# featureform/embeddinghub

Hardware: AMD Instinct MI355X
Metric: kNN queries/sec at recall@10>=0.95, 10Mx768 cosine, batch=1024 (higher is better)
Workload: dtype i8 filter -> f32 exact results; 1 GPU; 10000000x768 cosine (EHX-GAUSS-1), batch=1024, k=10, exact scan; rows=10000000, dims=768, batch=1024, k=10, rows_dtype=f32, world_size=1, parallelism=single GPU

## Files before the change

### embeddinghub_amd/csrc/ehx_env.h

```cpp
#pragma once
#include <cstdint>
#include <cstdlib>
#include <cstring>
#include <chrono>
#include <thread>

namespace ehx {

struct Env {
  bool scan_f32 = false;
  bool scan_f16 = false;
  uint64_t small_exact_bytes = 512ull << 20;
  bool one_launch = true;
  bool host_pipeline = true;
  bool allow_no_peer = false;
  uint32_t i8_growth = 0;
  double i8_safety = 2.0;
  int i8_sync = 0;
  long i8_kprime = 0;
  uint32_t i8_first_tiles = 0;
  uint64_t i8_first_keys = 0;
  uint32_t i8_width = 0;
  uint64_t i8_min_rows = 0;
  bool i8_sort = true;
  bool i8_trace = false;
  bool i8_count = false;
  bool i8_debug = false;
  bool i8_qres = true;
  bool i8_half = true;
  uint32_t stats_every = 2;
  bool i8_groupb = true;
  uint32_t i8_skew = 64;
  bool largek = true;
  uint32_t largek_growth = 4;
  uint32_t largek_min_queries = 0;
  bool rerank_staged = true;
  uint64_t build_div = 0;
  bool build_trace = false;
  long long build_scratch_keep = -1;
  bool graph_vislog = true;
  int graph_help = -1;
  uint32_t graph_width = 0;
  uint32_t test_pause_us = 0;
};

inline const Env& env() {
  static const Env e = [] {
    Env v;
    auto str = [](const char* n) { return getenv(n); };
    auto flag = [&](const char* n, bool dflt) {
      const char* g = str(n);
      return g ? atoi(g) != 0 : dflt;
    };
    if (const char* g = str("EHX_SCAN")) {
      v.scan_f32 = !strcmp(g, "f32");
// ... 27 lines not shown
    if (const char* g = str("EHX_I8_WIDTH")) {
      const long x = atol(g);
      if (x == 256 || x == 512 || x == 1024) v.i8_width = (uint32_t)x;
    }
    if (const char* g = str("EHX_I8_MIN_ROWS")) {
      const uint64_t x = strtoull(g, nullptr, 10);
      v.i8_min_rows = x < 4096 ? 4096 : x;
    }
    v.i8_sort = flag("EHX_I8_SORT", true);
    v.i8_trace = str("EHX_I8_TRACE") != nullptr;
    v.i8_count = str("EHX_I8_COUNT") != nullptr;
    v.i8_debug = str("EHX_I8_DEBUG") != nullptr;
    v.i8_qres = flag("EHX_I8_QRES", true);
    v.i8_half = flag("EHX_I8_HALF", true);
    v.i8_groupb = flag("EHX_I8_GROUPB", true);
    if (const char* g = str("EHX_STATS_EVERY")) {
      const long x = atol(g);
      v.stats_every = (uint32_t)(x < 1 ? 1 : (x > 1024 ? 1024 : x));
    }
    if (const char* g = str("EHX_I8_SKEW")) {
      const long x = atol(g);
      v.i8_skew = (uint32_t)(x < 0 ? 0 : (x > 4096 ? 4096 : x));
    }
    v.largek = flag("EHX_LARGEK", true);
    if (const char* g = str("EHX_LARGEK_GROWTH")) {
      const long x = atol(g);
      v.largek_growth = (uint32_t)(x < 2 ? 2 : (x > 16 ? 16 : x));
    }
    if (const char* g = str("EHX_LARGEK_MIN_QUERIES")) {
      const long x = atol(g);
      v.largek_min_queries = (uint32_t)(x < 1 ? 1 : (x > (1l << 24) ? (1l << 24) : x));
    }
    v.rerank_staged = flag("EHX_RERANK_STAGED", true);
    if (const char* g = str("EHX_BUILD_DIV")) {
      const long x = atol(g);
      v.build_div = (uint64_t)(x < 0 ? 0 : x);
    }
    v.build_trace = str("EHX_BUILD_TRACE") != nullptr;
    if (const char* g = str("EHX_BUILD_SCRATCH_KEEP")) v.build_scratch_keep = atoll(g);
    v.graph_vislog = flag("EHX_GRAPH_VISLOG", true);
    if (const char* g = str("EHX_GRAPH_HELP")) v.graph_help = atoi(g) != 0;
    if (const char* g = str("EHX_GRAPH_WIDTH")) {
      const long x = atol(g);
      if (x == 1 || x == 2 || x == 4) v.graph_width = (uint32_t)x;
    }
    if (const char* g = str("EHX_TEST_PAUSE_US")) {
// ... 14 lines not shown
```

### embeddinghub_amd/csrc/ehx_flat.cpp

```cpp
#include "ehx_internal.h"

namespace ehx_impl {

ScanPlan plan_scan(uint32_t nq, uint32_t n_tiles, uint32_t k, int n_cus) {
  ScanPlan p;
  p.q_tiles = (nq + kTileQ - 1) / kTileQ;
  p.q_rows = p.q_tiles * kTileQ;
  p.n_tiles = n_tiles;
  p.kprime = k + 8;
  uint32_t chunks = (uint32_t)n_cus / p.q_tiles;
  if (chunks < 1) chunks = 1;
  if (chunks >= 8) chunks &= ~7u;
  if (chunks > p.n_tiles) chunks = p.n_tiles ? p.n_tiles : 1;
  p.n_chunks = chunks;
  p.tiles_per_chunk = p.n_tiles ? (p.n_tiles + chunks - 1) / chunks : 0;
  p.grid = p.q_tiles * p.n_chunks;
  p.xcd_map = (p.n_chunks % 8 == 0) ? 1u : 0u;
  return p;
}

std::vector<ScanPass> plan_cascade(uint32_t nq, uint32_t n_tiles, uint32_t k, int n_cus, uint64_t first_tiles, uint64_t growth) {
  std::vector<ScanPass> passes;
  uint64_t done = 0;
  for (uint64_t cum = first_tiles; cum * 2 < n_tiles; cum *= growth) {
// ... 196 lines not shown
    const double f = (double)((uint64_t)(passes[i + 1].tile0) * kTileRows16) / (double)n_pub;
    return (uint32_t)std::min<double>(kprime, std::max<double>(16.0, std::ceil(kprime * f * safety)));
  };
  const uint64_t first_rows = (uint64_t)passes.front().plan.n_tiles * kTileRows16;
  const uint64_t first_keys_env = env().i8_first_keys;
  const uint64_t first_floor = first_keys_env ? first_keys_env : (big ? 64ull : std::min<uint64_t>(512, 2ull * kprime));
  const uint64_t first_keys = std::min<uint64_t>(
      2048, passes.size() == 1 ? 2ull * kprime : std::max<uint64_t>(first_floor, 2ull * rank_after(0)));
  const uint32_t sample_rank =
      (uint32_t)std::min<uint64_t>(64, std::max<uint64_t>(8, first_keys * kSampleTiles * kTileRows16 / first_rows));
  const ScanPlan p = passes.back().plan;
  test_pause();
  uint32_t grid_max = 0, chunks_max = 0;
  for (auto& ps : passes) {
    grid_max = std::max(grid_max, ps.plan.grid);
    chunks_max = std::max(chunks_max, ps.plan.n_chunks);
  }
  if (chunks_max > 256) return fail(EHX_EINTERNAL, "scan plan with %u chunks", chunks_max);
  int rc;
  ScanArgsI8 a;
  if ((rc = i8_scan_args(s, sc.buf, p, n_pub, &a))) return rc;
  if ((rc = sc.buf.dSample8.ensure((size_t)kSampleTiles * kTileRows16 * p.q_rows))) return rc;
  if ((rc = sc.buf.dMerged8.ensure((size_t)p.q_rows * width))) return rc;
  if ((rc = sc.buf.verdict.ensure(p.q_rows))) return rc;
  uint32_t* const pool_cnt = a.pool_cnt;
  uint32_t* const ovf = a.ovf;
  uint32_t* sync = sc.buf.dI8Ctl.p + 2 * (size_t)p.q_rows;
  if ((rc = wait_searches_in_flight(s, st))) return rc;
  if ((rc = sc.clock.begin(st, env().stats_every))) return rc;
  HIP_TRY(launch_prep_queries_i8(d_queries, (uint32_t)nq, s->dims, s->ld, s->ld8, p.q_rows, s->metric, sc.buf.dQ.p,
                                 sc.buf.dQ8.p, sc.buf.dQp8.p, sc.buf.dQuv.p, sc.buf.dThr8.p, sc.buf.dI8Ctl.p, st));
  auto scan = [&](const ScanPlan& pl, uint32_t tile0) -> hipError_t {
    set_scan_pass(a, pl, tile0);
    return launch_flat_scan_i8(a, st);
  };
  if ((rc = sc.clock.scan_begin(st))) return rc;
  {
    ScanPlan sp = plan_scan((uint32_t)nq, kSampleTiles, k, E.n_cus);
    a.dump = sc.buf.dSample8.p;
    a.sync = nullptr;
    HIP_TRY(scan(sp, 0));
    a.dump = nullptr;
    HIP_TRY(launch_sample_select256(sc.buf.dSample8.p, kSampleTiles * kTileRows16, p.q_rows, (uint32_t)nq, sample_rank,
                                    sc.buf.dThr8.p, st));
  }
  for (size_t i = 0; i < passes.size(); ++i) {
    const bool last = i + 1 == passes.size();
    a.sync = nullptr;
    if (use_sync && passes[i].plan.xcd_map && p.q_tiles > 1 && passes[i].plan.tiles_per_chunk >= 4 &&
        passes[i].plan.n_chunks * 4u <= kSyncWordsI8) {
      a.sync = sync;
      a.sync_tol = (uint32_t)sync_mode;
      if (i > 0) HIP_TRY(hipMemsetAsync(sync, 0, kSyncWordsI8 * sizeof(uint32_t), st));
    }
    HIP_TRY(scan(passes[i].plan, passes[i].tile0));
    if (last && (rc = sc.clock.scan_end(st))) return rc;
    HIP_TRY(launch_select256(sc.buf.dPool.p, pool_cnt, kPoolCap, (uint32_t)nq, rank_after(i), sc.buf.dMerged8.p, width, i > 0,
                             sc.buf.dThr8.p, sc.buf.dQp8.p, st));
  }
  Rerank256Args r;
  r.Q = sc.buf.dQ.p;
  r.X = s->rows.dX.p;
  r.x_half = (uint32_t)s->x_half;
  r.inv_norm = s->rows.dInv.p;
  r.merged = sc.buf.dMerged8.p;
  r.width = width;
  r.ovf = ovf;
  r.quv = sc.buf.dQuv.p;
  r.qparams = sc.buf.dQp8.p;
  r.max_sumsq = s->rows.dMaxSumsq.p;
  r.out_ids = d_ids;
  r.out_dist = d_dist;
  r.out_count = d_count;
  r.n_uncertified = sc.buf.verdict.count.p;
  r.uncert_flags = sc.buf.verdict.flags.p;
  r.nq = (uint32_t)nq;
// ... 76 lines not shown
  }
  s->i8_fb_score = 0;
  if (env().i8_trace)
    fprintf(stderr, "[ehx i8] %zu of %zu queries uncertified (%zu by a short list): candidate list now %u of %u\n", n_failed,
            nq, n_short, std::max(s->i8_kprime_min.load(), kprime), s->i8_width.load());
}

void count_scan_batch(ehx_space* s, size_t nq, uint64_t n_pub, uint32_t k, uint64_t elem_bytes) {
  s->n_queries += nq;
  s->n_dist += (uint64_t)nq * n_pub;
  s->bytes_algo += n_pub * s->dims * elem_bytes + (uint64_t)nq * s->dims * 4ull + (uint64_t)nq * k * 12ull;
}

int i8_stage_enqueue(ehx_space* s, uint64_t n_pub, int set, hipStream_t st, hipEvent_t after, bool pipelined, size_t nq,
                     const float* d_queries, uint32_t k, uint64_t* d_ids, float* d_dist, uint32_t* d_count, I8Outcome* o) {
  std::lock_guard<std::mutex> ql(s->i8_enqueue_mu);
  if (after) HIP_TRY(hipStreamWaitEvent(st, after, 0));
  int rc = flat_pass8(s, n_pub, set, st, nq, d_queries, k, d_ids, d_dist, d_count, &o->kprime);
  if (rc) return rc;
  Verdict& v = s->i8set[set].buf.verdict;
  return pipelined ? v.post_and_record(st) : v.post(st);
}

int i8_stage_outcome(ehx_space* s, uint64_t n_pub, int set, hipStream_t st, size_t nq, uint32_t k, I8Outcome* o) {
  Verdict& v = s->i8set[set].buf.verdict;
  o->failed.clear();
  o->n_short = 0;
  int rc;
  if (v.read() && (rc = v.collect(st, nq, nullptr, &o->failed, &o->n_short))) return rc;
  count_scan_batch(s, nq, n_pub, k, 1);
  s->n_i8_queries += nq;
  s->n_i8_fallback += o->failed.size();
  i8_adapt(s, nq, o->failed.size(), o->n_short, o->kprime);
  return EHX_OK;
}

int knn_device_locked(ehx_space* s, hipStream_t st, size_t nq, const float* d_queries, uint32_t k,
                      uint64_t* d_ids, float* d_dist, uint32_t* d_count, uint64_t n_pub) {
  if (k == 0 || nq == 0) return EHX_OK;
  if (nq > (1u << 24)) return fail(EHX_EINVAL, "too many queries in one call: %zu", nq);
  if (s->params.mode == EHX_MODE_GRAPH) {
    if (k > EHX_MAX_K_PAGED) return fail(EHX_EUNSUPPORTED, "graph mode: k=%u exceeds %u", k, EHX_MAX_K_PAGED);
    return knn_graph_locked(s, st, nq, d_queries, k, d_ids, d_dist, d_count);
  }
  if (n_pub == kNoSnapshot) n_pub = s->n.load(std::memory_order_acquire);
  if (k > EHX_MAX_K) {
    if (k > EHX_MAX_K_PAGED) return fail(EHX_EUNSUPPORTED, "k=%u exceeds EHX_MAX_K_PAGED=%u", k, EHX_MAX_K_PAGED);
    if (n_pub == 0) {
      HIP_TRY(hipMemsetAsync(d_count, 0, nq * sizeof(uint32_t), st));
      return EHX_OK;
// ... 90 lines not shown
```

### embeddinghub_amd/csrc/ehx_internal.h

```cpp
#pragma once
#include <hip/hip_runtime.h>

#include <algorithm>
#include <atomic>
#include <chrono>
#include <condition_variable>
#include <functional>
#include <map>
#include <random>
#include <set>
#include <cmath>
#include <cstdarg>
#include <cstdio>
#include <cstdlib>
#include <cstring>
#include <memory>
#include <mutex>
#include <shared_mutex>
#include <string>
#include <system_error>
#include <thread>
#include <unordered_map>
#include <vector>

#include "../../include/ehx.h"
#include "ehx_combine.h"
#include "ehx_env.h"
#include "ehx_kernels.h"

using namespace ehx;


struct ehx_space;

namespace ehx_impl {

extern thread_local char g_err[512];

int fail(int code, const char* fmt, ...);

#define HIP_TRY(expr)                                                                         \
  do {                                                                                        \
    hipError_t _e = (expr);                                                                   \
    if (_e != hipSuccess) {                                                                   \
      (void)hipGetLastError();                                                                \
      return fail(_e == hipErrorOutOfMemory ? EHX_ENOMEM : EHX_ENODEVICE, "%s failed: %s (%s:%d)", \
                  #expr, hipGetErrorString(_e), __FILE__, __LINE__);                          \
    }                                                                                         \
// ... 343 lines not shown
    DevBuf<uint64_t> dSample;
    RadiusKnnBufs scan;
    SubsetBufs group;
    HostStage host;
    DevBuf<unsigned long long> dCapHits;
    DevBuf<uint32_t> dWalkOf;
    SubsetBufs split;
  } masked;
  std::atomic<uint64_t> masked_ctr[5] = {};
  std::atomic<uint64_t> graphm_ctr[3] = {};
  RadiusKnnBufs largek;
  std::atomic<uint64_t> largek_ctr[5] = {};
  struct I8Set {
    struct Buffers {
      DevBuf<float> dQ;
      DevBuf<int8_t> dQ8;
      DevBuf<float4> dQp8;
      DevBuf<float2> dQuv;
      DevBuf<float> dThr8, dSample8;
      DevBuf<uint64_t> dPool, dMerged8;
      DevBuf<uint32_t> dI8Ctl;
      DevBuf<uint64_t> dCnt;
      Verdict verdict;
    } buf;
    BatchClock clock;
    std::mutex mu;
  };
  I8Set i8set[2];
  std::atomic<uint64_t> ev_counter{0};
  std::atomic<uint32_t> i8_next_set{0};
  std::mutex i8_enqueue_mu;
  std::atomic<uint64_t> n_filter_queries{0}, n_filter_fallback{0}, n_exhaustive{0}, n_uncertified_final{0};
  std::atomic<uint64_t> n_i8_queries{0}, n_i8_fallback{0};
  BatchClock clock;

  struct KnnReq : CombineReq {
    const float* q;
    size_t nq;
    uint32_t k;
    uint64_t* ids;
    float* dist;
    uint32_t* cnt;
  };
  Combiner<KnnReq> knn_combiner;
  std::atomic<uint64_t> n_coalesced_batches{0}, n_coalesced_queries{0};
  struct SetReq : CombineReq {
    const char* key;
    size_t klen;
    const float* vec;
  };
  Combiner<SetReq> set_combiner;
// ... 248 lines not shown
```

### embeddinghub_amd/csrc/ehx_kernels.h

```cpp
#pragma once

#include <hip/hip_fp16.h>
#include <hip/hip_runtime.h>
#include <atomic>
#include <stdint.h>

namespace ehx {

constexpr uint32_t kTileRows = 128;
constexpr uint32_t kTileQ = 256;
constexpr uint32_t kTileRows16 = 256;
constexpr uint32_t kBK = 32;
constexpr uint32_t kCandSlots = 64;
constexpr uint64_t kKeyInf = ~0ull;
constexpr uint32_t kNoNode = 0xFFFFFFFFu;

__host__ __device__ inline uint32_t f32_to_ordered(float f) {
#if defined(__HIP_DEVICE_COMPILE__)
  uint32_t u = __float_as_uint(f);
#else
  uint32_t u;
  __builtin_memcpy(&u, &f, 4);
#endif
  return u ^ ((u >> 31) ? 0xFFFFFFFFu : 0x80000000u);
// ... 149 lines not shown
  const float4* rowp;
  const float4* tilep;
  const float* tileg;
  const uint8_t* perm;
  const float4* qparams;
  const float* thr;
  float* dump = nullptr;
  uint64_t* cand;
  uint64_t* pool;
  uint32_t* pool_cnt;
  uint32_t* ovf;
  uint32_t pool_cap;
  uint32_t n;
  uint32_t ld;
  uint32_t tile0, n_tiles, q_tiles, n_chunks, tiles_per_chunk;
  uint32_t xcd_map;
  uint32_t* sync = nullptr;
  uint32_t sync_tol = 0;
  uint32_t skew = 0;
  uint32_t group_b = 0;
  const uint32_t* allow = nullptr;
  uint32_t allow_bits = 0;
  uint32_t allow_per_query = 0;
};
__host__ __device__ inline uint32_t scan8_swz(uint32_t rr) { return (0x78u >> (((rr >> 2) & 3u) * 2u)) & 3u; }
__host__ __device__ inline size_t scan8_index(uint64_t row, uint32_t col, uint32_t ld8) {
  const uint64_t tile = row >> 8;
  const uint32_t rr = (uint32_t)(row & 255u), kt = col >> 6, cc = col & 63u;
  const uint32_t chunk = (cc >> 4) ^ scan8_swz(rr);
  return ((size_t)(tile * (ld8 >> 6) + kt) * 256u + rr) * 64u + chunk * 16u + (cc & 15u);
}
__host__ __device__ inline size_t scanq8_index(uint64_t row, uint32_t stage, uint32_t cc, uint32_t ld8) {
  const uint64_t tile = row >> 8;
  const uint32_t rr = (uint32_t)(row & 255u);
  const uint32_t chunk = (cc >> 4) ^ scan8_swz(rr);
  return ((size_t)(tile * ((ld8 >> 6) + 3u) + stage) * 256u + rr) * 64u + chunk * 16u + (cc & 15u);
}
__host__ __device__ inline size_t scan8_dump_index(uint32_t q, uint32_t row, uint32_t n_s) {
  return ((((size_t)(q >> 4) * (n_s >> 4)) + (row >> 4)) << 8) + ((q & 15u) << 4) + (row & 15u);
}
inline size_t scanq8_bytes(uint32_t q_rows, uint32_t ld8) { return (size_t)(q_rows >> 8) * ((ld8 >> 6) + 3u) * 256u * 64u; }
constexpr size_t kScan8TailPadBytes = 3u * 256u * 64u;
size_t scan_i8_lds_bytes();
hipError_t launch_flat_scan_i8(const ScanArgsI8& a, hipStream_t st);
size_t make_scan8_scratch_bytes(uint64_t row0, uint64_t n, uint64_t sort_lo, uint64_t sort_hi);
hipError_t launch_make_scan8(const void* X, int x_half, uint64_t row0, uint64_t n, uint32_t dims, uint32_t ld,
// ... 337 lines not shown
```

### embeddinghub_amd/csrc/ehx_own.h

```cpp
#pragma once

namespace ehx_impl {

enum { kLiveDevice, kLivePinned, kLiveEvents, kLiveStreams };
inline std::atomic<uint64_t> g_live[4];

template <class T>
struct DevBuf {
  T* p = nullptr;
  size_t n = 0;
  DevBuf() = default;
  DevBuf(DevBuf&& o) noexcept { swap(o); }
  DevBuf& operator=(DevBuf&& o) noexcept {
    swap(o);
    return *this;
  }
  ~DevBuf() { release(); }
  void swap(DevBuf& o) noexcept {
    std::swap(p, o.p);
    std::swap(n, o.n);
  }
  int fresh(size_t want) {
    release();
    HIP_TRY(hipMalloc((void**)&p, want * sizeof(T)));
// ... 99 lines not shown
  }
  ~Stream() { release(); }
  operator hipStream_t() const { return s; }
  int ensure(unsigned flags) {
    if (s) return EHX_OK;
    HIP_TRY(hipStreamCreateWithFlags(&s, flags));
    g_live[kLiveStreams].fetch_add(1, std::memory_order_relaxed);
    return EHX_OK;
  }
  void release() {
    if (s) {
      (void)hipStreamDestroy(s);
      g_live[kLiveStreams].fetch_sub(1, std::memory_order_relaxed);
    }
    s = nullptr;
  }
};

struct Verdict {
  DevBuf<unsigned long long> count;
  DevBuf<uint32_t> flags;
  PinBuf<unsigned long long> landed;
  Event ev;

  int ensure(size_t q_rows) {
    int rc;
    if ((rc = count.ensure_zeroed_once(1)) || (rc = flags.ensure(q_rows))) return rc;
    return landed.ensure(1);
  }
  int post(hipStream_t st) {
    HIP_TRY(hipMemcpyAsync(landed.p, count.p, sizeof(unsigned long long), hipMemcpyDeviceToHost, st));
    return EHX_OK;
  }
  int post_and_record(hipStream_t st) {
    int rc;
    if ((rc = ev.ensure(hipEventBlockingSync | hipEventDisableTiming)) || (rc = post(st))) return rc;
    HIP_TRY(hipEventRecord(ev, st));
    return EHX_OK;
  }
  unsigned long long read() const {
#if defined(EHX_ABL) && EHX_ABL
    return 0;
#endif
    return *landed.p;
  }
  int collect(hipStream_t st, size_t m, const std::vector<uint32_t>* subset, std::vector<uint32_t>* out, size_t* n_short) {
    std::vector<uint32_t> f(m);
    HIP_TRY(hipMemsetAsync(count.p, 0, sizeof(unsigned long long), st));
    HIP_TRY(hipMemcpyAsync(f.data(), flags.p, m * sizeof(uint32_t), hipMemcpyDeviceToHost, st));
    HIP_TRY(hipStreamSynchronize(st));
    out->clear();
    *n_short = 0;
    for (size_t j = 0; j < m; ++j)
      if (f[j]) {
// ... 9 lines not shown
```

### embeddinghub_amd/csrc/ehx_testhooks.cpp

```cpp
#include "ehx_internal.h"

namespace {

enum { kArrX8, kArrRowp8, kArrTilep8, kArrTileg8, kArrPerm8, kArrUnsafe8, kArrLd8, kArrCap };
constexpr uint32_t kSampleTiles = 8;

int hook_space(ehx_space* s, const char* what, int need = 8) {
  int rc = ehx_init(nullptr, 0);
  if (rc) return rc;
  if (!valid_space(s)) return fail(EHX_EINVAL, "space is NULL");
  if (s->dropped) return fail(EHX_ENOTFOUND, "Not found");
  if (is_parent(s)) return fail(EHX_EUNSUPPORTED, "%s: space '%s' is row-sharded", what, s->name.c_str());
  if (need == 8 && !s->has8) return fail(EHX_EUNSUPPORTED, "%s: space '%s' keeps no int8 scan copy", what, s->name.c_str());
  if (need == 16 && !s->has16) return fail(EHX_EUNSUPPORTED, "%s: space '%s' keeps no fp16 scan copy", what, s->name.c_str());
  return EHX_OK;
}

template <class T>
int copy_slice(ehx_space* s, const ehx_impl::DevBuf<T>& b, uint64_t off, uint64_t n, void* out, hipStream_t st) {
  if (off > b.n || n > b.n - off) return fail(EHX_EINVAL, "slice [%llu, +%llu) of an array of %llu elements",
                                              (unsigned long long)off, (unsigned long long)n, (unsigned long long)b.n);
  if (n == 0) return EHX_OK;
  HIP_TRY(hipMemcpyAsync(out, b.p + off, n * sizeof(T), hipMemcpyDeviceToHost, st));
  return sync_stream(s, st);
// ... 231 lines not shown
    (void)hipGetLastError();
    return rc;
  }
  out_info[0] = p.q_rows;
  out_info[1] = s->ld8;
  out_info[3] = p.n_chunks;
  out_info[4] = p.tiles_per_chunk;
  out_info[5] = p.xcd_map;
  out_info[6] = (uint32_t)n_pub;
  out_info[7] = lockstep;
  if (thr) {
    for (size_t q = 0; q < nq; ++q) {
      const size_t m = std::min<size_t>(out_cnt[q], kPoolCap);
      for (size_t i = 0; i < kPoolCap; ++i) {
        const uint64_t key = i < m ? pool[q * kPoolCap + i] : kKeyInf;
        out_ids[q * kPoolCap + i] = (uint32_t)key;
        out_scores[q * kPoolCap + i] = i < m ? ordered_to_f32((uint32_t)(key >> 32)) : __builtin_inff();
      }
    }
  }
  return EHX_OK;
}

int ehx_test_f16_array(ehx_space* s, int which, uint64_t elem_offset, uint64_t n_elems, void* out) {
  int rc = hook_space(s, "ehx_test_f16_array", 16);
  if (rc) return rc;
  if (!out && n_elems) return fail(EHX_EINVAL, "NULL argument");
  std::lock_guard<std::mutex> wl(s->wmu);
  std::shared_lock<std::shared_mutex> rl(s->mu);
  if (s->dropped) return fail(EHX_ENOTFOUND, "Not found");
  HIP_TRY(hipSetDevice(s->device));
  const hipStream_t ws = s->wr.wstream ? (hipStream_t)s->wr.wstream : (hipStream_t)s->stream;
  if ((rc = sync_stream(s, ws)) || (rc = sync_stream(s, s->stream))) return rc;
  switch (which) {
    case kArrX16: return copy_slice(s, s->f16.dX16, elem_offset, n_elems, out, ws);
    case kArrUnsafe16: return copy_slice(s, s->f16.dUnsafe, elem_offset, n_elems, out, ws);
    case kArrRowp16: {
      const DevBuf<float2>& b = s->f16.dRowp16;
      if (elem_offset > b.n * 2 || n_elems > b.n * 2 - elem_offset) return fail(EHX_EINVAL, "slice beyond the array");
      if (n_elems == 0) return EHX_OK;
      HIP_TRY(hipMemcpyAsync(out, (const float*)b.p + elem_offset, n_elems * sizeof(float), hipMemcpyDeviceToHost, ws));
      return sync_stream(s, ws);
    }
    case kArrLd16:
    case kArrCap16:
      if (elem_offset != 0 || n_elems != 1) return fail(EHX_EINVAL, "a scalar: offset 0, one element");
// ... 75 lines not shown
```

### embeddinghub_amd/csrc/k_flati8.hip

```cpp
#include "ehx_env.h"
#include "ehx_kernels.h"
#include "k_scan_common.h"

namespace ehx {

typedef int i32x4 __attribute__((ext_vector_type(4)));

namespace {

constexpr uint32_t kRingI8 = 4;
constexpr uint32_t kRowBI8 = 64;
constexpr uint32_t kStageI8 = kTileRows16 * kRowBI8;
template <bool HALF>
struct I8L {
  static constexpr int kThreads = HALF ? 256 : 512;
  static constexpr uint32_t kWaves = HALF ? 4 : 8;
  static constexpr uint32_t kXStage = HALF ? kStageI8 / 2 : kStageI8;
  static constexpr uint32_t kXShift = HALF ? 13 : 14;
  static constexpr uint32_t kQSlots = HALF ? 2 : kRingI8;
  static constexpr uint32_t kStgCap = HALF ? 64 : 128;
  static constexpr uint32_t kRowpSlot = (HALF ? 128 : 256) * 16;
  static constexpr uint32_t kRowpWaves = HALF ? 2 : 4;
  static constexpr uint32_t kXOff = 0;
  static constexpr uint32_t kQOff = kRingI8 * kXStage;
// ... 112 lines not shown
  if (m == 0ull) return;
  const uint32_t k = (uint32_t)__builtin_popcountll(m);
  uint32_t* cnt = (uint32_t*)(smem + L::kStgCntOff) + w;
  if (stg_n + k > L::kStgCap) {
    if ((threadIdx.x & 63) == 0) *cnt = stg_n;
    asm volatile("s_waitcnt lgkmcnt(0)" ::: "memory");
    i8_flush_staging<HALF, MASKED>();
    stg_n = 0u;
  }
  if (hi) {
    const uint32_t pos = stg_n + __builtin_amdgcn_mbcnt_hi((uint32_t)(m >> 32), __builtin_amdgcn_mbcnt_lo((uint32_t)m, 0u));
    uint64_t* keys = (uint64_t*)(smem + L::kStgKeyOff) + (size_t)w * L::kStgCap;
    uint32_t* qls = (uint32_t*)(smem + L::kStgQlOff) + (size_t)w * L::kStgCap;
    keys[pos] = ((uint64_t)(uint32_t)v << 32) | (uint64_t)(tile_row0 + r_local);
    qls[pos] = (uint32_t)ql;
  }
  stg_n += k;
}

}

size_t scan_i8_lds_bytes() { return I8L<false>::kLdsBytes; }

template <bool DUMP, bool REV, bool QRES = false, bool HALF = false, bool PAIR = false, int MASKED = kMaskNone>
__global__ __launch_bounds__(I8L<HALF>::kThreads, 2) void flat_scan_i8_kernel(const ScanArgsI8 a) {
  static_assert(!QRES || (!REV && !DUMP), "QRES: the run-time-slot loop of the plain scan only");
  static_assert(!PAIR || (!REV && !DUMP && !QRES && !HALF), "PAIR: the run-time-slot loop of the plain scan, stages in pairs");
  static_assert(!HALF || QRES, "HALF: short rows, the query tile resident in LDS");
  static_assert(!MASKED || !DUMP, "MASKED: the flush of a collecting scan");
  using L = I8L<HALF>;
  extern __shared__ __attribute__((aligned(16))) char smem[];
  const int tid = threadIdx.x;
  const int lane = tid & 63;
  const int w = __builtin_amdgcn_readfirstlane(tid >> 6);
  const int j15 = lane & 15, qd = lane >> 4;

  uint32_t qt, chunk, half = 0u;
  {
    uint32_t b = blockIdx.x;
    if (a.xcd_map) {
      const uint32_t xcd = b & 7u;
      uint32_t slot = b >> 3;
      if constexpr (HALF) {
        half = slot & 1u;
        slot >>= 1;
      }
      qt = slot % a.q_tiles;
      chunk = xcd * (a.n_chunks >> 3) + slot / a.q_tiles;
// ... 17 lines not shown
  if (tid < (int)kTileQ) {
    const size_t qg = (size_t)qt * kTileQ + tid;
    float4 qp = a.qparams[qg];
    qp.w = a.thr ? a.thr[qg] : __builtin_inff();
    qp_lds[tid] = qp;
    qinv_lds[tid] = qp.x > 0.0f ? (1.0f - 1e-5f) / qp.x : __builtin_inff();
  }
  if (tid < 64) ((uint32_t*)(smem + L::kSyncOff))[tid] = 0u;
  if (tid < 8) ((uint32_t*)(smem + L::kStgCntOff))[tid] = 0u;
  if (tid == 0) {
    I8Ctx* ctx = (I8Ctx*)(smem + L::kCtxOff);
    ctx->pool = a.pool;
    ctx->pool_cnt = a.pool_cnt;
    ctx->ovf = a.ovf;
    ctx->perm = a.perm;
    ctx->rowp = a.rowp;
    ctx->pool_cap = a.pool_cap;
    ctx->n = a.n;
    ctx->q_tile0 = qt * kTileQ;
    ctx->allow_bits = MASKED ? a.allow_bits : 0u;
    if constexpr (MASKED) ctx->allow = a.allow;
  }

  const uint32_t tile_begin = a.tile0 + chunk * a.tiles_per_chunk;
  uint32_t tile_end = tile_begin + a.tiles_per_chunk;
  if (tile_end > a.tile0 + a.n_tiles) tile_end = a.tile0 + a.n_tiles;
  const uint32_t my_tiles =
      (uint32_t)__builtin_amdgcn_readfirstlane((int)(tile_end > tile_begin ? tile_end - tile_begin : 0u));
  const uint32_t ktiles = a.ld / kRowBI8;

  const uint32_t voff = (uint32_t)lane * 16u;
  const uint32_t voff8 = voff + L::kXStage / 2;
  const size_t tile_bytes = (size_t)ktiles * kStageI8;
  const char* xsrc = (const char*)a.X + (size_t)tile_begin * tile_bytes + (size_t)half * L::kXStage * (HALF ? 1u : 0u) +
                     (size_t)w * 1024;
  const char* qbase = (const char*)a.Q + (size_t)qt * ((size_t)(ktiles + 3) * kStageI8) + (size_t)w * 1024;
  const char* qsrc = qbase;
  const uint32_t rpiece = (uint32_t)w & (L::kRowpWaves - 1u);
  const char* rsrc = (const char*)(a.rowp + (size_t)tile_begin * kTileRows16 + (HALF ? (size_t)half * 128u : 0u)) +
                     (size_t)rpiece * 1024;
  const uint32_t xdst = L::kXOff + (uint32_t)w * 1024u;
  const uint32_t qdst = L::kQOff + (uint32_t)w * 1024u;
  const uint32_t rdst = L::kRowpOff + rpiece * 1024u;

#define EHX_DMA(DST_BASE, DST_IMM, VOFF, SRC)                                                              \
  do {                                                                                                     \
    asm volatile("s_add_u32 m0, %0, %1\n\ts_nop 0\n\tglobal_load_lds_dwordx4 %2, %3"                       \
                 :                                                                                         \
                 : "s"(DST_BASE), "n"(DST_IMM), "v"(VOFF), "s"(SRC)                                        \
// ... 167 lines not shown

  uint32_t* const sync_ctr = (a.sync && a.sync_tol > 0u && a.xcd_map && a.q_tiles > 1 && REV && a.q_tiles <= 4)
                                 ? a.sync + chunk * 4u
                                 : nullptr;
  bool sync_on = sync_ctr != nullptr && !DUMP && !HALF;
  const uint32_t sync_m0 = L::kSyncOff;

  __syncthreads();
#if EHX_I8_PRIO
  {
    uint32_t hwid_p;
    asm volatile("s_getreg_b32 %0, hwreg(HW_REG_HW_ID)" : "=s"(hwid_p));
    if (hwid_p & 1u) __builtin_amdgcn_s_setprio(1);
  }
#endif
  if constexpr (HALF) {
    if (a.skew && my_tiles >= 16u) {
      uint32_t hwid;
      asm volatile("s_getreg_b32 %0, hwreg(HW_REG_HW_ID)" : "=s"(hwid));
      if (hwid & 1u) {
        for (uint32_t i = 32; i <= a.skew; i += 32) __builtin_amdgcn_s_sleep(32);
        for (uint32_t i = 0; i < (a.skew & 31u); ++i) __builtin_amdgcn_s_sleep(1);
      }
    }
  }
  if (my_tiles > 0) {
  if (DUMP && w < (int)L::kRowpWaves) EHX_DMA(rdst, 0, voff, rsrc);
  constexpr int kStageWait = QRES ? 4 : 8;
  if constexpr (QRES) {
    for (uint32_t ks = 0; ks < ktiles; ++ks) {
      const uint32_t qd0 = qdst + (ks << 14);
      constexpr uint32_t kQStep = HALF ? 4096u : 8192u;
#pragma unroll
      for (uint32_t pc = 0; pc < 16u / L::kWaves; ++pc) {
        const uint32_t qdp = qd0 + pc * kQStep, vo = voff + pc * kQStep;
        asm volatile("s_mov_b32 m0, %0\n\ts_nop 0\n\tglobal_load_lds_dwordx4 %1, %2" : : "s"(qdp), "v"(vo), "s"(qsrc) : "memory");
      }
      qsrc += kStageI8;
    }
    EHX_DMA_X0(0); EHX_DMA_X1(0); xsrc += kStageI8;
    EHX_DMA_X0(1); EHX_DMA_X1(1); xsrc += kStageI8;
    EHX_DMA_X0(2); EHX_DMA_X1(2); xsrc += kStageI8;
  } else {
    EHX_DMA_X0(0); EHX_DMA_Q0(0); EHX_DMA_X1(0); EHX_DMA_Q1(0);
    EHX_DMA_X0(1); EHX_DMA_Q0(1); EHX_DMA_X1(1); EHX_DMA_Q1(1);
    EHX_DMA_X0(2); EHX_DMA_Q0(2); EHX_DMA_X1(2); EHX_DMA_Q1(2);
// ... 269 lines not shown
#undef EHX_SB
#undef EHX_FR
#undef EHX_SDMA
#undef EHX_DMA_RT
#undef EHX_SDMA_X0
#undef EHX_SDMA_Q0
#undef EHX_SDMA_X1
#undef EHX_SDMA_Q1
#undef EHX_STAGE16_CT
#undef EHX_STAGE16_BODY
#undef EHX_STAGE_BARRIER
#undef EHX_MFZ
#undef EHX_DMA_X0
#undef EHX_DMA_Q0
#undef EHX_DMA_X1
#undef EHX_DMA_Q1
#undef EHX_DMA

  asm volatile("s_waitcnt vmcnt(0) lgkmcnt(0)" ::: "memory");
  if (DUMP) return;
  if (lane == 0) ((uint32_t*)(smem + L::kStgCntOff))[w] = stg_n;
  asm volatile("s_waitcnt lgkmcnt(0)" ::: "memory");
  i8_flush_staging<HALF, MASKED>();
}

hipError_t launch_flat_scan_i8(const ScanArgsI8& a, hipStream_t st) {
  static DynLdsAttr attr;
  const void* fns[] = {(const void*)flat_scan_i8_kernel<false, true>, (const void*)flat_scan_i8_kernel<false, false>,
                       (const void*)flat_scan_i8_kernel<true, true>, (const void*)flat_scan_i8_kernel<true, false>,
                       (const void*)flat_scan_i8_kernel<false, false, true>,
                       (const void*)flat_scan_i8_kernel<false, false, true, true>,
                       (const void*)flat_scan_i8_kernel<false, false, false, false, true>,
                       (const void*)flat_scan_i8_kernel<false, true, false, false, false, true>,
                       (const void*)flat_scan_i8_kernel<false, false, false, false, false, true>,
                       (const void*)flat_scan_i8_kernel<false, false, true, false, false, true>,
                       (const void*)flat_scan_i8_kernel<false, false, true, true, false, true>,
                       (const void*)flat_scan_i8_kernel<false, false, false, false, true, true>,
                       (const void*)flat_scan_i8_kernel<false, true, false, false, false, kMaskPerQuery>,
                       (const void*)flat_scan_i8_kernel<false, false, false, false, false, kMaskPerQuery>,
                       (const void*)flat_scan_i8_kernel<false, false, true, false, false, kMaskPerQuery>,
                       (const void*)flat_scan_i8_kernel<false, false, true, true, false, kMaskPerQuery>,
                       (const void*)flat_scan_i8_kernel<false, false, false, false, true, kMaskPerQuery>};
  if (hipError_t e = attr.ensure(fns, (int)(sizeof(fns) / sizeof(fns[0])), I8L<false>::kLdsBytes); e != hipSuccess) return e;
  if (a.ld == 0 || a.ld % kRowBI8) return hipErrorInvalidValue;
  const uint32_t grid = a.q_tiles * a.n_chunks;
  const bool rev = a.ld % (4 * kRowBI8) == 0;
#define EHX_LAUNCH_I8(D, R) \
  hipLaunchKernelGGL((flat_scan_i8_kernel<D, R>), dim3(grid), dim3(I8L<false>::kThreads), I8L<false>::kLdsBytes, st, a)
  const bool qres_on = env().i8_qres;
  if (a.allow) {
    if (a.dump) return hipErrorInvalidValue;
#define EHX_LAUNCH_I8_MASKED(M)                                                                                              \
  do {                                                                                                                       \
    if (rev)                                                                                                                 \
      hipLaunchKernelGGL((flat_scan_i8_kernel<false, true, false, false, false, M>), dim3(grid), dim3(I8L<false>::kThreads), \
                         I8L<false>::kLdsBytes, st, a);                                                                      \
    else if (qres_on && env().i8_half && a.ld <= 2 * kRowBI8)                                                                \
      hipLaunchKernelGGL((flat_scan_i8_kernel<false, false, true, true, false, M>), dim3(2 * grid),                          \
                         dim3(I8L<true>::kThreads), I8L<true>::kLdsBytes, st, a);                                            \
    else if (qres_on && a.ld <= 4 * kRowBI8)                                                                                 \
      hipLaunchKernelGGL((flat_scan_i8_kernel<false, false, true, false, false, M>), dim3(grid), dim3(I8L<false>::kThreads), \
                         I8L<false>::kLdsBytes, st, a);                                                                      \
    else if ((a.ld / kRowBI8) % 2u == 0u)                                                                                    \
      hipLaunchKernelGGL((flat_scan_i8_kernel<false, false, false, false, true, M>), dim3(grid), dim3(I8L<false>::kThreads), \
                         I8L<false>::kLdsBytes, st, a);                                                                      \
    else                                                                                                                     \
      hipLaunchKernelGGL((flat_scan_i8_kernel<false, false, false, false, false, M>), dim3(grid),                            \
                         dim3(I8L<false>::kThreads), I8L<false>::kLdsBytes, st, a);                                          \
  } while (0)
    if (a.allow_per_query) EHX_LAUNCH_I8_MASKED(kMaskPerQuery);
    else EHX_LAUNCH_I8_MASKED(kMaskOne);
#undef EHX_LAUNCH_I8_MASKED
  } else if (a.dump) {
    if (rev) EHX_LAUNCH_I8(true, true);
    else EHX_LAUNCH_I8(true, false);
  } else {
    const bool half_on = env().i8_half;
    if (rev) EHX_LAUNCH_I8(false, true);
    else if (qres_on && half_on && a.ld <= 2 * kRowBI8)
      hipLaunchKernelGGL((flat_scan_i8_kernel<false, false, true, true>), dim3(2 * grid), dim3(I8L<true>::kThreads),
                         I8L<true>::kLdsBytes, st, a);
    else if (qres_on && a.ld <= 4 * kRowBI8)
      hipLaunchKernelGGL((flat_scan_i8_kernel<false, false, true>), dim3(grid), dim3(I8L<false>::kThreads), I8L<false>::kLdsBytes, st, a);
    else if ((a.ld / kRowBI8) % 2u == 0u)
      hipLaunchKernelGGL((flat_scan_i8_kernel<false, false, false, false, true>), dim3(grid), dim3(I8L<false>::kThreads),
                         I8L<false>::kLdsBytes, st, a);
    else EHX_LAUNCH_I8(false, false);
  }
#undef EHX_LAUNCH_I8
  return hipGetLastError();
}

}
```

Measured before the change: 167,900 queries/s.

## Adaptively rebalance i8 scan tile ranges across XCDs from per-block timestamps

Adds a feedback balancer for the reversed-layout i8 scan. Each block records start and finish wall-clock stamps, which ride back to the host with the verdict count copy. Per-XCD throughput is derived from these stamps and smoothed per launch shape, then used to size per-chunk tile ranges in a pinned bounds table that later launches read. The aim is to cut tail time when some XCDs run slower than others. The cost is extra stamp writes and memory waits in the kernel, a larger device-to-host copy, and host bookkeeping.

```diff
diff --git a/embeddinghub_amd/csrc/ehx_balance.h b/embeddinghub_amd/csrc/ehx_balance.h
--- /dev/null
+++ b/embeddinghub_amd/csrc/ehx_balance.h
@@ -0,0 +1,156 @@
+#pragma once
+#include <algorithm>
+#include <cmath>
+#include <cstdint>
+#include <cstring>
+#include <mutex>
+
+namespace ehx {
+
+constexpr uint32_t kXcds = 8;
+constexpr uint32_t kBalanceMaxChunks = 256;
+constexpr double kBalanceLo = 0.85, kBalanceHi = 1.15;
+constexpr double kBalanceGain = 0.25;
+
+inline void balance_uniform(uint32_t n_tiles, uint32_t n_chunks, uint32_t* bounds) {
+  const uint64_t tpc = n_chunks ? ((uint64_t)n_tiles + n_chunks - 1) / n_chunks : 0;
+  for (uint32_t c = 0; c <= n_chunks; ++c) bounds[c] = (uint32_t)std::min<uint64_t>((uint64_t)c * tpc, n_tiles);
+}
+
+inline bool balance_valid(const uint32_t* bounds, uint32_t n_tiles, uint32_t n_chunks) {
+  if (n_chunks == 0 || n_chunks > kBalanceMaxChunks || bounds[0] != 0u || bounds[n_chunks] != n_tiles) return false;
+  for (uint32_t c = 0; c < n_chunks; ++c)
+    if (bounds[c] > bounds[c + 1]) return false;
+  return true;
+}
+
+inline bool balance_bounds(const double* f, uint32_t n_tiles, uint32_t n_chunks, uint32_t* bounds) {
+  bool ok = n_chunks > 0 && n_chunks <= kBalanceMaxChunks && n_chunks % kXcds == 0;
+  double sum = 0.0;
+  for (uint32_t x = 0; ok && x < kXcds; ++x) {
+    ok = std::isfinite(f[x]) && f[x] >= 0.0;
+    sum += f[x];
+  }
+  ok = ok && std::isfinite(sum) && sum > 0.0;
+  if (ok) {
+    const uint32_t cpx = n_chunks / kXcds;
+    double cum = 0.0;
+    uint32_t lo = 0;
+    for (uint32_t x = 0; x < kXcds; ++x) {
+      cum += f[x];
+      uint32_t hi = x + 1 == kXcds ? n_tiles : (uint32_t)std::min<double>((double)n_tiles, std::floor((double)n_tiles * (cum / sum) + 0.5));
+      if (hi < lo) hi = lo;
+      const uint64_t len = hi - lo;
+      for (uint32_t j = 0; j < cpx; ++j) bounds[x * cpx + j] = lo + (uint32_t)(len * j / cpx);
+      lo = hi;
+    }
+    bounds[n_chunks] = n_tiles;
+    ok = balance_valid(bounds, n_tiles, n_chunks);
+  }
+  if (!ok) balance_uniform(n_tiles, n_chunks, bounds);
+  return ok;
+}
+
+inline void balance_xcd_tiles(const uint32_t* bounds, uint32_t n_chunks, uint32_t* tiles) {
+  const uint32_t cpx = n_chunks / kXcds;
+  for (uint32_t x = 0; x < kXcds; ++x) tiles[x] = bounds[(x + 1) * cpx] - bounds[x * cpx];
+}
+
+inline bool balance_rates(const uint64_t* stamps, uint32_t grid, const uint32_t* tiles, double* rate, uint64_t* t0_out = nullptr,
+                          uint64_t* finish_out = nullptr) {
+  uint64_t t0 = ~0ull, fin[kXcds] = {0, 0, 0, 0, 0, 0, 0, 0};
+  for (uint32_t b = 0; b < grid; ++b) {
+    t0 = std::min(t0, stamps[2 * b]);
+    fin[b & 7u] = std::max(fin[b & 7u], stamps[2 * b + 1]);
+  }
+  if (t0_out) *t0_out = t0;
+  double sum = 0.0;
+  uint32_t n = 0;
+  for (uint32_t x = 0; x < kXcds; ++x) {
+    if (finish_out) finish_out[x] = fin[x];
+    rate[x] = 0.0;
+    if (tiles[x] == 0 || fin[x] <= t0) continue;
+    rate[x] = (double)tiles[x] / (double)(fin[x] - t0);
+    sum += rate[x];
+    ++n;
+  }
+  if (n == 0 || !(sum > 0.0)) return false;
+  for (uint32_t x = 0; x < kXcds; ++x) rate[x] *= (double)n / sum;
+  return true;
+}
+
+struct BalanceState {
+  static constexpr int kShapes = 4;
+  struct Shape {
+    uint64_t key = 0;
+    double f[kXcds];
+    uint64_t updates = 0, used = 0;
+  };
+
+  static uint64_t key_of(uint32_t q_tiles, uint32_t n_chunks, uint32_t tiles_per_chunk) {
+    uint32_t cls = 0;
+    while ((tiles_per_chunk >> cls) > 1u) ++cls;
+    return 1ull | ((uint64_t)q_tiles << 8) | ((uint64_t)n_chunks << 24) | ((uint64_t)cls << 40);
+  }
+
+  void factors(uint64_t key, double* out) {
+    std::lock_guard<std::mutex> l(mu);
+    if (forced) {
+      std::copy(forced_f, forced_f + kXcds, out);
+      return;
+    }
+    const Shape* s = find(key);
+    for (uint32_t x = 0; x < kXcds; ++x) out[x] = s && s->updates ? s->f[x] : 1.0;
+  }
+  void update(uint64_t key, const double* rate) {
+    std::lock_guard<std::mutex> l(mu);
+    if (forced) return;
+    Shape* s = find(key);
+    if (!s) {
+      s = &shape[0];
+      for (Shape& c : shape)
+        if (c.key == 0 || (s->key != 0 && c.used < s->used)) s = &c;
+      s->key = key;
+      s->updates = 0;
+      for (double& v : s->f) v = 1.0;
+    }
+    for (uint32_t x = 0; x < kXcds; ++x) {
+      if (!(rate[x] > 0.0) || !std::isfinite(rate[x])) continue;
+      const double v = s->updates ? s->f[x] + kBalanceGain * (rate[x] - s->f[x]) : rate[x];
+      s->f[x] = std::min(kBalanceHi, std::max(kBalanceLo, v));
+    }
+    ++s->updates;
+    s->used = ++tick;
+  }
+  void force(const double* f) {
+    std::lock_guard<std::mutex> l(mu);
+    forced = f != nullptr;
+    if (f) std::copy(f, f + kXcds, forced_f);
+  }
+  bool is_forced() {
+    std::lock_guard<std::mutex> l(mu);
+    return forced;
+  }
+  void reset() {
+    std::lock_guard<std::mutex> l(mu);
+    for (Shape& c : shape) c = Shape();
+    forced = false;
+  }
+
+ private:
+  Shape* find(uint64_t key) {
+    for (Shape& c : shape)
+      if (c.key == key) {
+        c.used = ++tick;
+        return &c;
+      }
+    return nullptr;
+  }
+  std::mutex mu;
+  Shape shape[kShapes];
+  uint64_t tick = 0;
+  bool forced = false;
+  double forced_f[kXcds] = {1, 1, 1, 1, 1, 1, 1, 1};
+};
+
+}
diff --git a/embeddinghub_amd/csrc/ehx_env.h b/embeddinghub_amd/csrc/ehx_env.h
--- a/embeddinghub_amd/csrc/ehx_env.h
+++ b/embeddinghub_amd/csrc/ehx_env.h
@@ -31,6 +31,7 @@
   uint32_t stats_every = 2;
   bool i8_groupb = true;
   uint32_t i8_skew = 64;
+  bool i8_balance = true;
   bool largek = true;
   uint32_t largek_growth = 4;
   uint32_t largek_min_queries = 0;
@@ -104,6 +105,7 @@
       const long x = atol(g);
       v.i8_skew = (uint32_t)(x < 0 ? 0 : (x > 4096 ? 4096 : x));
     }
+    v.i8_balance = flag("EHX_I8_BALANCE", true);
     v.largek = flag("EHX_LARGEK", true);
     if (const char* g = str("EHX_LARGEK_GROWTH")) {
       const long x = atol(g);
diff --git a/embeddinghub_amd/csrc/ehx_flat.cpp b/embeddinghub_amd/csrc/ehx_flat.cpp
--- a/embeddinghub_amd/csrc/ehx_flat.cpp
+++ b/embeddinghub_amd/csrc/ehx_flat.cpp
@@ -242,7 +242,39 @@
   if ((rc = i8_scan_args(s, sc.buf, p, n_pub, &a))) return rc;
   if ((rc = sc.buf.dSample8.ensure((size_t)kSampleTiles * kTileRows16 * p.q_rows))) return rc;
   if ((rc = sc.buf.dMerged8.ensure((size_t)p.q_rows * width))) return rc;
-  if ((rc = sc.buf.verdict.ensure(p.q_rows))) return rc;
+  if ((rc = sc.buf.verdict.ensure(p.q_rows, ehx_space::I8Set::kStampWords))) return rc;
+  constexpr uint32_t kTable = kBalanceMaxChunks + 1;
+  std::vector<int> stamp_slot(passes.size(), -1);
+  sc.n_stamped = 0;
+  if (s->ld8 % 256u == 0u && !s->keyless) {
+    const uint32_t min_tpc = s->i8_balance_min_tpc.load(std::memory_order_relaxed);
+    uint32_t off = 0;
+    for (size_t i = passes.size(); i-- > 0 && sc.n_stamped < ehx_space::I8Set::kStampedPasses;) {
+      const ScanPlan& pl = passes[i].plan;
+      if (!pl.xcd_map || pl.tiles_per_chunk < min_tpc || pl.grid > ehx_space::I8Set::kStampGrid || pl.n_chunks > kBalanceMaxChunks)
+        continue;
+      ehx_space::I8Set::StampedPass& sp = sc.stamped[sc.n_stamped];
+      sp.key = BalanceState::key_of(pl.q_tiles, pl.n_chunks, pl.tiles_per_chunk);
+      sp.grid = pl.grid;
+      sp.q_tiles = pl.q_tiles;
+      sp.n_tiles = pl.n_tiles;
+      sp.n_chunks = pl.n_chunks;
+      sp.tile0 = passes[i].tile0;
+      sp.stamp_off = off;
+      off += 2 * pl.grid;
+      double f[kXcds];
+      s->i8_balance.factors(sp.key, f);
+      sp.table = env().i8_balance && balance_bounds(f, pl.n_tiles, pl.n_chunks, sp.bounds);
+      if (!sp.table) balance_uniform(pl.n_tiles, pl.n_chunks, sp.bounds);
+      stamp_slot[i] = (int)sc.n_stamped++;
+    }
+    if (sc.n_stamped &&
+        (rc = sc.buf.hBounds.ensure((size_t)ehx_space::I8Set::kStampedPasses * kTable, hipHostMallocCoherent | hipHostMallocMapped, true)))
+      return rc;
+    sc.buf.verdict.riding = off;
+  } else {
+    sc.buf.verdict.riding = 0;
+  }
   uint32_t* const pool_cnt = a.pool_cnt;
   uint32_t* const ovf = a.ovf;
   uint32_t* sync = sc.buf.dI8Ctl.p + 2 * (size_t)p.q_rows;
@@ -272,6 +304,17 @@
       a.sync = sync;
       a.sync_tol = (uint32_t)sync_mode;
       if (i > 0) HIP_TRY(hipMemsetAsync(sync, 0, kSyncWordsI8 * sizeof(uint32_t), st));
+    }
+    a.bounds = nullptr;
+    a.stamps = nullptr;
+    if (stamp_slot[i] >= 0) {
+      const ehx_space::I8Set::StampedPass& sp = sc.stamped[stamp_slot[i]];
+      a.stamps = (uint64_t*)sc.buf.verdict.extra_dev() + sp.stamp_off;
+      if (sp.table) {
+        uint32_t* const tab = sc.buf.hBounds.p + (size_t)stamp_slot[i] * kTable;
+        std::copy(sp.bounds, sp.bounds + sp.n_chunks + 1, tab);
+        a.bounds = tab;
+      }
     }
     HIP_TRY(scan(passes[i].plan, passes[i].tile0));
     if (last && (rc = sc.clock.scan_end(st))) return rc;
@@ -394,10 +437,40 @@
   return pipelined ? v.post_and_record(st) : v.post(st);
 }
 
+static void i8_balance_outcome(ehx_space* s, ehx_space::I8Set& sc) {
+  const uint64_t* const words = (const uint64_t*)sc.buf.verdict.extra_landed();
+  for (uint32_t j = sc.n_stamped; j-- > 0;) {
+    const ehx_space::I8Set::StampedPass& sp = sc.stamped[j];
+    const uint64_t* const stamps = words + sp.stamp_off;
+    uint32_t tiles[kXcds];
+    double rate[kXcds];
+    balance_xcd_tiles(sp.bounds, sp.n_chunks, tiles);
+    const bool ok = balance_rates(stamps, sp.grid, tiles, rate);
+    if (ok) s->i8_balance.update(sp.key, rate);
+    if (j == 0) {
+      ehx_space::I8BalanceLast& l = s->i8_balance_last;
+      std::lock_guard<std::mutex> g(l.mu);
+      ++l.batches;
+      l.grid = sp.grid;
+      l.q_tiles = sp.q_tiles;
+      l.n_tiles = sp.n_tiles;
+      l.n_chunks = sp.n_chunks;
+      l.tile0 = sp.tile0;
+      l.table = sp.table ? 1u : 0u;
+      std::copy(sp.bounds, sp.bounds + sp.n_chunks + 1, l.bounds);
+      l.stamps.assign(stamps, stamps + 2 * (size_t)sp.grid);
+      s->i8_balance.factors(sp.key, l.factors);
+      std::copy(rate, rate + kXcds, l.rate);
+    }
+  }
+  sc.n_stamped = 0;
+}
+
 int i8_stage_outcome(ehx_space* s, uint64_t n_pub, int set, hipStream_t st, size_t nq, uint32_t k, I8Outcome* o) {
   Verdict& v = s->i8set[set].buf.verdict;
   o->failed.clear();
   o->n_short = 0;
+  i8_balance_outcome(s, s->i8set[set]);
   int rc;
   if (v.read() && (rc = v.collect(st, nq, nullptr, &o->failed, &o->n_short))) return rc;
   count_scan_batch(s, nq, n_pub, k, 1);
diff --git a/embeddinghub_amd/csrc/ehx_internal.h b/embeddinghub_amd/csrc/ehx_internal.h
--- a/embeddinghub_amd/csrc/ehx_internal.h
+++ b/embeddinghub_amd/csrc/ehx_internal.h
@@ -24,6 +24,7 @@
 #include <vector>
 
 #include "../../include/ehx.h"
+#include "ehx_balance.h"
 #include "ehx_combine.h"
 #include "ehx_env.h"
 #include "ehx_kernels.h"
@@ -413,11 +414,32 @@
       DevBuf<uint32_t> dI8Ctl;
       DevBuf<uint64_t> dCnt;
       Verdict verdict;
+      PinBuf<uint32_t> hBounds;
     } buf;
     BatchClock clock;
     std::mutex mu;
+    static constexpr uint32_t kStampedPasses = 2, kStampGrid = 512;
+    static constexpr size_t kStampWords = (size_t)kStampedPasses * 2 * kStampGrid;
+    struct StampedPass {
+      uint64_t key;
+      uint32_t grid, q_tiles, n_tiles, n_chunks, tile0;
+      uint32_t stamp_off;
+      bool table;
+      uint32_t bounds[kBalanceMaxChunks + 1];
+    } stamped[kStampedPasses];
+    uint32_t n_stamped = 0;
   };
   I8Set i8set[2];
+  BalanceState i8_balance;
+  std::atomic<uint32_t> i8_balance_min_tpc{64};
+  struct I8BalanceLast {
+    std::mutex mu;
+    uint64_t batches = 0;
+    uint32_t grid = 0, q_tiles = 0, n_tiles = 0, n_chunks = 0, tile0 = 0, table = 0;
+    uint32_t bounds[kBalanceMaxChunks + 1] = {};
+    std::vector<uint64_t> stamps;
+    double factors[kXcds] = {}, rate[kXcds] = {};
+  } i8_balance_last;
   std::atomic<uint64_t> ev_counter{0};
   std::atomic<uint32_t> i8_next_set{0};
   std::mutex i8_enqueue_mu;
diff --git a/embeddinghub_amd/csrc/ehx_kernels.h b/embeddinghub_amd/csrc/ehx_kernels.h
--- a/embeddinghub_amd/csrc/ehx_kernels.h
+++ b/embeddinghub_amd/csrc/ehx_kernels.h
@@ -195,6 +195,8 @@
   const uint32_t* allow = nullptr;
   uint32_t allow_bits = 0;
   uint32_t allow_per_query = 0;
+  const uint32_t* bounds = nullptr;
+  uint64_t* stamps = nullptr;
 };
 __host__ __device__ inline uint32_t scan8_swz(uint32_t rr) { return (0x78u >> (((rr >> 2) & 3u) * 2u)) & 3u; }
 __host__ __device__ inline size_t scan8_index(uint64_t row, uint32_t col, uint32_t ld8) {
diff --git a/embeddinghub_amd/csrc/ehx_own.h b/embeddinghub_amd/csrc/ehx_own.h
--- a/embeddinghub_amd/csrc/ehx_own.h
+++ b/embeddinghub_amd/csrc/ehx_own.h
@@ -145,14 +145,18 @@
   DevBuf<uint32_t> flags;
   PinBuf<unsigned long long> landed;
   Event ev;
+  size_t riding = 0;
 
-  int ensure(size_t q_rows) {
+  int ensure(size_t q_rows, size_t extra = 0) {
     int rc;
-    if ((rc = count.ensure_zeroed_once(1)) || (rc = flags.ensure(q_rows))) return rc;
-    return landed.ensure(1);
+    if ((rc = count.ensure_zeroed_once(1 + extra)) || (rc = flags.ensure(q_rows))) return rc;
+    return landed.ensure(1 + extra);
   }
+  unsigned long long* extra_dev() const { return count.p + 1; }
+  const unsigned long long* extra_landed() const { return landed.p + 1; }
   int post(hipStream_t st) {
-    HIP_TRY(hipMemcpyAsync(landed.p, count.p, sizeof(unsigned long long), hipMemcpyDeviceToHost, st));
+    const size_t words = 1 + std::min(riding, count.n ? count.n - 1 : 0);
+    HIP_TRY(hipMemcpyAsync(landed.p, count.p, words * sizeof(unsigned long long), hipMemcpyDeviceToHost, st));
     return EHX_OK;
   }
   int post_and_record(hipStream_t st) {
diff --git a/embeddinghub_amd/csrc/ehx_testhooks.cpp b/embeddinghub_amd/csrc/ehx_testhooks.cpp
--- a/embeddinghub_amd/csrc/ehx_testhooks.cpp
+++ b/embeddinghub_amd/csrc/ehx_testhooks.cpp
@@ -277,6 +277,43 @@
   return EHX_OK;
 }
 
+int ehx_test_i8_balance_force(ehx_space* s, const double* f8, uint32_t min_tiles_per_chunk) {
+  int rc = hook_space(s, "ehx_test_i8_balance_force");
+  if (rc) return rc;
+  if (f8) {
+    double sum = 0.0;
+    for (uint32_t x = 0; x < kXcds; ++x) {
+      if (!(f8[x] >= 0.0) || !std::isfinite(f8[x])) return fail(EHX_EINVAL, "factor %u is not a non-negative number", x);
+      sum += f8[x];
+    }
+    if (!(sum > 0.0)) return fail(EHX_EINVAL, "all factors are zero");
+    s->i8_balance.force(f8);
+  } else {
+    s->i8_balance.reset();
+  }
+  s->i8_balance_min_tpc.store(min_tiles_per_chunk ? min_tiles_per_chunk : 64u, std::memory_order_relaxed);
+  return EHX_OK;
+}
+
+int ehx_test_i8_balance_read(ehx_space* s, uint64_t* out_info, uint32_t* out_bounds, uint64_t* out_stamps, double* out_factors,
+                             double* out_rates) {
+  int rc = hook_space(s, "ehx_test_i8_balance_read");
+  if (rc) return rc;
+  if (!out_info || !out_bounds || !out_stamps || !out_factors || !out_rates) return fail(EHX_EINVAL, "NULL argument");
+  int khz = 0;
+  HIP_TRY(hipDeviceGetAttribute(&khz, hipDeviceAttributeWallClockRate, s->device));
+  ehx_space::I8BalanceLast& l = s->i8_balance_last;
+  std::lock_guard<std::mutex> g(l.mu);
+  if (l.batches == 0) return fail(EHX_ENOTFOUND, "no stamped pass yet");
+  const uint64_t info[8] = {l.batches, l.grid, l.q_tiles, l.n_tiles, l.n_chunks, l.tile0, l.table, (uint64_t)khz};
+  std::copy(info, info + 8, out_info);
+  std::copy(l.bounds, l.bounds + l.n_chunks + 1, out_bounds);
+  std::copy(l.stamps.begin(), l.stamps.end(), out_stamps);
+  std::copy(l.factors, l.factors + kXcds, out_factors);
+  std::copy(l.rate, l.rate + kXcds, out_rates);
+  return EHX_OK;
+}
+
 int ehx_test_f16_array(ehx_space* s, int which, uint64_t elem_offset, uint64_t n_elems, void* out) {
   int rc = hook_space(s, "ehx_test_f16_array", 16);
   if (rc) return rc;
diff --git a/embeddinghub_amd/csrc/k_flati8.hip b/embeddinghub_amd/csrc/k_flati8.hip
--- a/embeddinghub_amd/csrc/k_flati8.hip
+++ b/embeddinghub_amd/csrc/k_flati8.hip
@@ -158,8 +158,9 @@
 
 size_t scan_i8_lds_bytes() { return I8L<false>::kLdsBytes; }
 
-template <bool DUMP, bool REV, bool QRES = false, bool HALF = false, bool PAIR = false, int MASKED = kMaskNone>
+template <bool DUMP, bool REV, bool QRES = false, bool HALF = false, bool PAIR = false, int MASKED = kMaskNone, bool TAB = false>
 __global__ __launch_bounds__(I8L<HALF>::kThreads, 2) void flat_scan_i8_kernel(const ScanArgsI8 a) {
+  static_assert(!TAB || (REV && !DUMP && !QRES && !HALF && !PAIR && !MASKED), "TAB: the plain compile-time-slot scan only");
   static_assert(!QRES || (!REV && !DUMP), "QRES: the run-time-slot loop of the plain scan only");
   static_assert(!PAIR || (!REV && !DUMP && !QRES && !HALF), "PAIR: the run-time-slot loop of the plain scan, stages in pairs");
   static_assert(!HALF || QRES, "HALF: short rows, the query tile resident in LDS");
@@ -223,9 +224,22 @@
     if constexpr (MASKED) ctx->allow = a.allow;
   }
 
-  const uint32_t tile_begin = a.tile0 + chunk * a.tiles_per_chunk;
+  uint32_t tile_begin = a.tile0 + chunk * a.tiles_per_chunk;
   uint32_t tile_end = tile_begin + a.tiles_per_chunk;
   if (tile_end > a.tile0 + a.n_tiles) tile_end = a.tile0 + a.n_tiles;
+  if constexpr (TAB) {
+    if (a.bounds) {
+      typedef const __attribute__((address_space(4))) uint32_t* cu32p;
+      const uint64_t bv = (uint64_t)(a.bounds + chunk);
+      const uint32_t blo = (uint32_t)__builtin_amdgcn_readfirstlane((int)(uint32_t)bv);
+      const uint32_t bhi = (uint32_t)__builtin_amdgcn_readfirstlane((int)(uint32_t)(bv >> 32));
+      const cu32p bp = (cu32p)(((uint64_t)bhi << 32) | blo);
+      tile_begin = a.tile0 + bp[0];
+      tile_end = a.tile0 + bp[1];
+      if (tile_end > a.tile0 + a.n_tiles) tile_end = a.tile0 + a.n_tiles;
+      if (tile_begin > tile_end) tile_begin = tile_end;
+    }
+  }
   const uint32_t my_tiles =
       (uint32_t)__builtin_amdgcn_readfirstlane((int)(tile_end > tile_begin ? tile_end - tile_begin : 0u));
   const uint32_t ktiles = a.ld / kRowBI8;
@@ -439,6 +453,12 @@
         for (uint32_t i = 32; i <= a.skew; i += 32) __builtin_amdgcn_s_sleep(32);
         for (uint32_t i = 0; i < (a.skew & 31u); ++i) __builtin_amdgcn_s_sleep(1);
       }
+    }
+  }
+  if constexpr (TAB) {
+    if (a.stamps) {
+      if (tid == 0) a.stamps[2u * blockIdx.x] = wall_clock64();
+      asm volatile("s_waitcnt vmcnt(0)" ::: "memory");
     }
   }
   if (my_tiles > 0) {
@@ -754,6 +774,12 @@
   if (lane == 0) ((uint32_t*)(smem + L::kStgCntOff))[w] = stg_n;
   asm volatile("s_waitcnt lgkmcnt(0)" ::: "memory");
   i8_flush_staging<HALF, MASKED>();
+  if constexpr (TAB) {
+    if (a.stamps) {
+      __syncthreads();
+      if (tid == 0) a.stamps[2u * blockIdx.x + 1u] = wall_clock64();
+    }
+  }
 }
 
 hipError_t launch_flat_scan_i8(const ScanArgsI8& a, hipStream_t st) {
@@ -772,7 +798,8 @@
                        (const void*)flat_scan_i8_kernel<false, false, false, false, false, kMaskPerQuery>,
                        (const void*)flat_scan_i8_kernel<false, false, true, false, false, kMaskPerQuery>,
                        (const void*)flat_scan_i8_kernel<false, false, true, true, false, kMaskPerQuery>,
-                       (const void*)flat_scan_i8_kernel<false, false, false, false, true, kMaskPerQuery>};
+                       (const void*)flat_scan_i8_kernel<false, false, false, false, true, kMaskPerQuery>,
+                       (const void*)flat_scan_i8_kernel<false, true, false, false, false, kMaskNone, true>};
   if (hipError_t e = attr.ensure(fns, (int)(sizeof(fns) / sizeof(fns[0])), I8L<false>::kLdsBytes); e != hipSuccess) return e;
   if (a.ld == 0 || a.ld % kRowBI8) return hipErrorInvalidValue;
   const uint32_t grid = a.q_tiles * a.n_chunks;
@@ -808,7 +835,11 @@
     else EHX_LAUNCH_I8(true, false);
   } else {
     const bool half_on = env().i8_half;
-    if (rev) EHX_LAUNCH_I8(false, true);
+    if (rev && (a.bounds || a.stamps))
+      hipLaunchKernelGGL((flat_scan_i8_kernel<false, true, false, false, false, kMaskNone, true>), dim3(grid),
+                         dim3(I8L<false>::kThreads), I8L<false>::kLdsBytes, st, a);
+    else if (a.bounds || a.stamps) return hipErrorInvalidValue;
+    else if (rev) EHX_LAUNCH_I8(false, true);
     else if (qres_on && half_on && a.ld <= 2 * kRowBI8)
       hipLaunchKernelGGL((flat_scan_i8_kernel<false, false, true, true>), dim3(2 * grid), dim3(I8L<true>::kThreads),
                          I8L<true>::kLdsBytes, st, a);
```

Result: faster. 171,100 queries/s, median of 6 (+1.9%).
